# zoltanmaric/h264-fer

Hardware: AMD Instinct MI355X
Metric: macroblocks/sec encode (1080p full-search ME) + bit-exact bitstream vs ref (higher is better)
Workload: dtype u8; 1 GPU; 1080p IPPP encode, full-search +-16 ME (BASELINE configs[2]); content=textured, coded_size=1920x1072, streams_per_gpu=256, contexts_per_gpu=1, gop=30, qp=12, window=32, maxdiff=3, parallelism=1 x 256 independent closed-GOP streams

## Files before the change

### h264-fer_amd/csrc/fer_me.hip

```cpp
#include <stdlib.h>
#include "fer_internal.h"
#include "fer_mvpred.h"

#define INF_M 1000000000

struct WList {
    int m;
    int xy;
};

__device__ __forceinline__ int pack_xy(int x, int y) { return (x & 0xffff) | (y << 16); }
__device__ __forceinline__ int unp_x(int xy) { return (int)(short)(xy & 0xffff); }
__device__ __forceinline__ int unp_y(int xy) { return xy >> 16; }

__device__ __forceinline__ void wl_insert(WList &L, int K, int lane, bool valid, int m, int xy)
{
    int thr = lane_bcast(L.m, K - 1);
    unsigned long long mask = __ballot(valid && m < thr);
    while (mask) {
        int src = __ffsll((long long)mask) - 1;
        mask &= mask - 1;
        int cm = lane_bcast(m, src), cxy = lane_bcast(xy, src);
        int pos = __popcll(__ballot(lane < K && L.m <= cm));
        if (pos < K) {
            int um = FER_DPP(L.m, DPP_WAVE_SHR1), uxy = FER_DPP(L.xy, DPP_WAVE_SHR1);
            if (lane > pos && lane < K) {
                L.m = um;
                L.xy = uxy;
            } else if (lane == pos) {
                L.m = cm;
                L.xy = cxy;
            }
        }
    }
}

#define WAVE_LDS_SYNC()                                    \
    do {                                                   \
        __builtin_amdgcn_fence(__ATOMIC_SEQ_CST, "wavefront"); \
        __builtin_amdgcn_wave_barrier();                   \
    } while (0)
__device__ __forceinline__ int lds_rank64(const unsigned *p, unsigned mine, int n4 = 16)
{
    const uint4 *q = (const uint4 *)p;
    int r = 0;
#pragma unroll 4
    for (int i = 0; i < n4; i++) {
        uint4 k = q[i];
        r += (int)(k.x < mine) + (int)(k.y < mine) + (int)(k.z < mine) + (int)(k.w < mine);
    }
    return r;
}

template <int NB, bool ORDERED, class RAW, class FIN, class ARR>
__device__ __forceinline__ bool select_topk_ex(const int (&v)[NB], int K, int lane, int *sel, WList &L, RAW raw, FIN fin, ARR arr)
{
    unsigned *A = (unsigned *)sel, *B = A + 64;
    int *Ci = sel + 128, *Di = sel + 192;
    const unsigned long long lt = (1ull << lane) - 1ull;
    int lmin = 0x7fffffff, lmax = -1, total = 0;
#pragma unroll
    for (int u = 0; u < NB; u++) {
        total += __popcll(__ballot(v[u] >= 0));
        lmin = (int)min((unsigned)lmin, (unsigned)v[u]);
        lmax = max(lmax, v[u]);
    }
    const int need = min(K, total);
    L.m = INF_M;
    L.xy = 0;
    if (need == 0) return true;
    int c = 65;
    if (!__any(lmax >= (1 << 26))) {
        B[lane] = 0xffffffffu;
        int T0 = 0x7fffffff;
        if (__popcll(__ballot(lmin != 0x7fffffff)) >= need) {
            int lo = 0, hi = (1 << 21) - 1;
            if (__popcll(__ballot(lmin <= hi)) >= need) {
                while (lo < hi) {
                    const int mid = (lo + hi) >> 1;
                    if (__popcll(__ballot(lmin <= mid)) >= need)
                        hi = mid;
                    else
                        lo = mid + 1;
                }
                T0 = lo;
            } else {
                T0 = 1 << 21;
            }
        }
        WAVE_LDS_SYNC();
        if (T0 < (1 << 21) && NB * 64 <= 2048) {
            int nsurv = 0;
#pragma unroll
            for (int u = 0; u < NB; u++) {
                const bool take = (unsigned)v[u] <= (unsigned)T0;
                const unsigned long long mk = __ballot(take);
                if (mk) {
                    const int slot = nsurv + (int)__builtin_amdgcn_mbcnt_hi((uint32_t)(mk >> 32), __builtin_amdgcn_mbcnt_lo((uint32_t)mk, 0u));
                    if (take && slot < 64) {
                        B[slot] = ((unsigned)v[u] << 11) | (unsigned)arr(u);
                        Ci[slot] = raw(u);
                    }
                    nsurv += __popcll(mk);
                }
            }
            WAVE_LDS_SYNC();
            c = nsurv;
        }
    }
    if (c <= 64) {
        WAVE_LDS_SYNC();
        const unsigned mine = B[lane];
        const int mypay = Ci[lane];
        const int rk = lds_rank64(B, mine, (__builtin_amdgcn_readfirstlane(c) + 3) >> 2);
        WAVE_LDS_SYNC();
        if (lane < c && rk < need) {
            A[rk] = mine >> 11;
            Di[rk] = mypay;
        }
        WAVE_LDS_SYNC();
        if (lane < need) {
            L.m = (int)A[lane];
            L.xy = fin(Di[lane]);
        }
        WAVE_LDS_SYNC();
        return true;
    }
    if (!ORDERED) return false;
    int *key = sel, *kxy = sel + 64, *key2 = sel + 128, *kxy2 = sel + 192;
    int lo = wave_min(lmin), hi;
    if (__popcll(__ballot(lmin != 0x7fffffff)) >= need)
        hi = wave_max(lmin != 0x7fffffff ? lmin : -1);
    else
        hi = wave_max(lmax);
    while (lo < hi) {
        int mid = lo + ((hi - lo) >> 1);
        int cnt = 0;
#pragma unroll
        for (int u = 0; u < NB; u++) cnt += __popcll(__ballot(v[u] >= 0 && v[u] <= mid));
        if (cnt >= need)
            hi = mid;
        else
            lo = mid + 1;
    }
    const int T = lo;
    int c_less = 0;
#pragma unroll
    for (int u = 0; u < NB; u++) c_less += __popcll(__ballot(v[u] >= 0 && v[u] < T));
    const int take_eq = need - c_less;
    int nsel = 0, eq_seen = 0;
    WAVE_LDS_SYNC();
#pragma unroll
    for (int u = 0; u < NB; u++) {
        bool ok = v[u] >= 0;
        bool eq = ok && v[u] == T;
        unsigned long long meq = __ballot(eq);
        bool take = (ok && v[u] < T) || (eq && eq_seen + __popcll(meq & lt) < take_eq);
        unsigned long long mt = __ballot(take);
        if (take) {
            int pos = nsel + __popcll(mt & lt);
            key[pos] = v[u];
            kxy[pos] = raw(u);
        }
        nsel += __popcll(mt);
        eq_seen += __popcll(meq);
    }
    WAVE_LDS_SYNC();
    int mk = lane < need ? key[lane] : INF_M, mxy = lane < need ? kxy[lane] : 0;
    int rank = 0;
    for (int i = 0; i < need; i++) {
        int ki = key[i];
        rank += (ki < mk) || (ki == mk && i < lane);
    }
    if (lane < need) {
        key2[rank] = mk;
        kxy2[rank] = mxy;
    }
    WAVE_LDS_SYNC();
    if (lane < need) {
        L.m = key2[lane];
        L.xy = fin(kxy2[lane]);
    }
    WAVE_LDS_SYNC();
    return true;
}
template <int NB, class RAW, class FIN>
__device__ __forceinline__ void select_topk(const int (&v)[NB], int K, int lane, int *sel, WList &L, RAW raw, FIN fin)
{
    select_topk_ex<NB, true>(v, K, lane, sel, L, raw, fin, [&](int u) { return u * 64 + lane; });
}

typedef unsigned short u16x2_t __attribute__((ext_vector_type(2)));
typedef short i16x2_t __attribute__((ext_vector_type(2)));
__device__ __forceinline__ uint32_t pk_sub16(uint32_t a, uint32_t b)
{
    return __builtin_bit_cast(uint32_t, (u16x2_t)(__builtin_bit_cast(u16x2_t, a) - __builtin_bit_cast(u16x2_t, b)));
}
__device__ __forceinline__ uint32_t pk_abs16(uint32_t a)
{
    i16x2_t x = __builtin_bit_cast(i16x2_t, a), z = {0, 0};
    return __builtin_bit_cast(uint32_t, __builtin_elementwise_max(x, (i16x2_t)(z - x)));
}
struct SuPk {
    uint32_t s01, s23, s4;
    uint32_t d01, d23, d4;
    uint32_t s12, s34;
    uint32_t e12, e34;
};
__device__ __forceinline__ SuPk su_pack(const int s[5])
{
    SuPk p;
    p.s01 = (uint32_t)s[0] | ((uint32_t)s[1] << 16);
    p.s23 = (uint32_t)s[2] | ((uint32_t)s[3] << 16);
    p.s4 = (uint32_t)s[4];
    p.d01 = (uint32_t)(s[0] - s[1]) << 16;
    p.d23 = (uint32_t)(s[0] - s[2]) | ((uint32_t)(s[0] - s[3]) << 16);
    p.d4 = (uint32_t)(s[0] - s[4]);
    p.s12 = (uint32_t)s[1] | ((uint32_t)s[2] << 16);
    p.s34 = (uint32_t)s[3] | ((uint32_t)s[4] << 16);
    p.e12 = (uint32_t)(s[0] - s[1]) | ((uint32_t)(s[0] - s[2]) << 16);
    p.e34 = (uint32_t)(s[0] - s[3]) | ((uint32_t)(s[0] - s[4]) << 16);
    return p;
}
__device__ __forceinline__ int feat_dist_w(uint32_t a, uint32_t b, uint32_t c, const SuPk &p)
{
    uint32_t t = __builtin_amdgcn_sad_u16(a, p.s01, 0);
    t = __builtin_amdgcn_sad_u16(b, p.s23, t);
    t = __builtin_amdgcn_sad_u16(c, p.s4, t);
    uint32_t kk = __builtin_amdgcn_perm(a, a, 0x01000100);
    t = __builtin_amdgcn_sad_u16(pk_sub16(kk, a), p.d01, t);
    t = __builtin_amdgcn_sad_u16(pk_sub16(kk, b), p.d23, t);
    t = __builtin_amdgcn_sad_u16(pk_sub16(kk, c) & 0xffffu, p.d4, t);
    return (int)t;
}
__device__ __forceinline__ int feat_dist_rec(const uint16_t *__restrict__ rec, const SuPk &p)
{
    const uint32_t *r = (const uint32_t *)rec;
    return feat_dist_w(r[0], r[1], r[2], p);
}
struct FeatRec {
    uint32_t a, b, c;
};

__device__ __forceinline__ FeatRec feat_rec_direct(const IPlanes &ip, int W, int H, int frac, int refy, int refx)
{
    const int y = iclamp(refy, 0, H - 1), x = iclamp(refx, 0, W - 1);
    const uint8_t *p0 = ip.base + (size_t)frac * ip.plane + (size_t)y * ip.pitch + (x & ~3);
    const uint32_t sh = (uint32_t)(x & 3);
    uint32_t h84[8], hc[8];
#pragma unroll
    for (int r = 0; r < 8; r++) {
        const uint32_t *w = (const uint32_t *)(p0 + (size_t)r * ip.pitch);
        const uint32_t lo = __builtin_amdgcn_alignbyte(w[1], w[0], sh), hi = __builtin_amdgcn_alignbyte(w[2], w[1], sh);
        const uint32_t a4 = __builtin_amdgcn_sad_u8(lo, 0u, 0u);
        h84[r] = __builtin_amdgcn_sad_u8(hi, 0u, a4) | (a4 << 16);
        hc[r] = __builtin_amdgcn_udot4(hi, 0x00000101u, __builtin_amdgcn_udot4(lo, 0x00000101u, 0u, false), false);
    }
    const uint32_t top = h84[0] + h84[1] + h84[2] + h84[3], all = top + h84[4] + h84[5] + h84[6] + h84[7];
    const uint32_t k3 = (h84[0] + h84[1] + h84[4] + h84[5]) & 0xffffu;
    const uint32_t k4 = hc[0] + hc[1] + hc[2] + hc[3] + hc[4] + hc[5] + hc[6] + hc[7];
    FeatRec f;
    f.a = (all & 0xffffu) | (top << 16);
    f.b = (all >> 16) | (k3 << 16);
    f.c = k4;
    return f;
}

template <int R1>
struct LocalGeo {
    static constexpr int N1 = 2 * R1 + 1, PW = 2 * R1 + 8, NC = N1 * N1 * 16, NB = (NC + 63) / 64;
    static constexpr int HTAB = 8 * PW * N1 * 2;
};
template <int R1>
struct LocalLoads {
    static constexpr int ROUNDS = (8 * LocalGeo<R1>::PW + 63) / 64;
    uint4 w[2][ROUNDS];
};
template <int R1>
__device__ __forceinline__ void local_request(const IPlanes &ip, int W, int H, int px0, int py0, int lane, LocalLoads<R1> &ld)
{
    using G = LocalGeo<R1>;
    constexpr int N1 = G::N1, PW = G::PW;
#pragma unroll
    for (int half = 0; half < 2; half++)
#pragma unroll
        for (int k = 0; k < LocalLoads<R1>::ROUNDS; k++) ld.w[half][k] = make_uint4(0, 0, 0, 0);
    if (px0 + N1 - 1 < 0 || px0 >= W || py0 + N1 - 1 < 0 || py0 >= H) return;
    const uint8_t *mbase = ip.base - ((size_t)FER_IP_T * ip.pitch + FER_IP_L);
    const uint32_t obase = __umul24((uint32_t)(py0 + FER_IP_T), (uint32_t)ip.pitch) + (uint32_t)((px0 & ~3) + FER_IP_L);
#pragma unroll
    for (int half = 0; half < 2; half++) {
#pragma unroll
        for (int k = 0; k < LocalLoads<R1>::ROUNDS; k++) {
            const int tt = min(k * 64 + lane, 8 * PW - 1);
            const int fl = tt / PW, r = tt - fl * PW;
            typedef uint32_t u32x4_a4 __attribute__((ext_vector_type(4), aligned(4)));
            const u32x4_a4 v = *(const u32x4_a4 *)(mbase + (obase + __umul24((uint32_t)(half * 8 + fl), (uint32_t)ip.plane) + __umul24((uint32_t)r, (uint32_t)ip.pitch)));
            ld.w[half][k] = make_uint4(v.x, v.y, v.z, v.w);
        }
    }
}
template <int R1>
__device__ __forceinline__ void local_metrics(const IPlanes &ip, int W, int H, int px0, int py0, const SuPk &sp, int lane,
                                              uint32_t *htab, int *mtab, int half_lo = 0, int half_hi = 2, const LocalLoads<R1> *pre = nullptr)
{
    using G = LocalGeo<R1>;
    constexpr int N1 = G::N1, PW = G::PW;
    static_assert(PW + 3 <= 16, "the patch row must fit one 16-byte load");
    if (px0 + N1 - 1 < 0 || px0 >= W || py0 + N1 - 1 < 0 || py0 >= H) {
#pragma unroll
        for (int u = 0; u < G::NB; u++) mtab[u * 64 + lane] = -1;
        WAVE_LDS_SYNC();
        return;
    }
    const uint32_t sh = (uint32_t)(px0 & 3);
    const uint8_t *mbase = ip.base - ((size_t)FER_IP_T * ip.pitch + FER_IP_L);
    const uint32_t obase = __umul24((uint32_t)(py0 + FER_IP_T), (uint32_t)ip.pitch) + (uint32_t)((px0 & ~3) + FER_IP_L);
    for (int half = half_lo; half < half_hi; half++) {
#pragma unroll
        for (int t0 = 0; t0 < 8 * PW; t0 += 64) {
            const int t = t0 + lane;
            const int tt = min(t, 8 * PW - 1);
            const int fl = tt / PW, r = tt - fl * PW;
            typedef uint32_t u32x4_a4 __attribute__((ext_vector_type(4), aligned(4)));
            uint4 w;
            if (pre) {
                w = half == 0 ? pre->w[0][t0 / 64] : pre->w[1][t0 / 64];
            } else {
                const u32x4_a4 v = *(const u32x4_a4 *)(mbase + (obase + __umul24((uint32_t)(half * 8 + fl), (uint32_t)ip.plane) + __umul24((uint32_t)r, (uint32_t)ip.pitch)));
                w = make_uint4(v.x, v.y, v.z, v.w);
            }
            const uint32_t b0 = __builtin_amdgcn_alignbyte(w.y, w.x, sh), b1 = __builtin_amdgcn_alignbyte(w.z, w.y, sh),
                           b2 = __builtin_amdgcn_alignbyte(w.w, w.z, sh);
            if (t < 8 * PW) {
                uint32_t *o = htab + (size_t)tt * N1 * 2;
#pragma unroll
                for (int ix = 0; ix < N1; ix++) {
                    const uint32_t lo = ix < 4 ? __builtin_amdgcn_alignbyte(b1, b0, (uint32_t)(ix & 3)) : b1;
                    const uint32_t hi = ix < 4 ? __builtin_amdgcn_alignbyte(b2, b1, (uint32_t)(ix & 3)) : b2;
                    const uint32_t a4 = __builtin_amdgcn_sad_u8(lo, 0u, 0u);
                    o[ix * 2] = __builtin_amdgcn_sad_u8(hi, 0u, a4) | (a4 << 16);
                    o[ix * 2 + 1] = __builtin_amdgcn_udot4(hi, 0x00000101u, __builtin_amdgcn_udot4(lo, 0x00000101u, 0u, false), false);
                }
            }
        }
        WAVE_LDS_SYNC();
        if (lane < 8 * N1) {
            const int fl = lane / N1, ix = lane - fl * N1;
            uint32_t P84[PW + 1], Pc[PW + 1];
            P84[0] = 0;
            Pc[0] = 0;
#pragma unroll
            for (int r = 0; r < PW; r++) {
                const uint2 h = *(const uint2 *)(htab + ((size_t)(fl * PW + r) * N1 + ix) * 2);
                P84[r + 1] = P84[r] + h.x;
                Pc[r + 1] = Pc[r] + h.y;
            }
            const int refx = px0 + ix, wx = iabs(ix - R1) + 4;
            const bool xok = refx >= 0 && refx < W;
#pragma unroll
            for (int iy = 0; iy < N1; iy++) {
                const uint32_t all = P84[iy + 8] - P84[iy];
                const uint32_t k1 = (P84[iy + 4] - P84[iy]) & 0xffffu;
                const uint32_t k3 = ((P84[iy + 2] - P84[iy]) + (P84[iy + 6] - P84[iy + 4])) & 0xffffu;
                const uint32_t k4 = Pc[iy + 8] - Pc[iy];
                const int D = feat_dist_w((all & 0xffffu) | (k1 << 16), (all >> 16) | (k3 << 16), k4, sp);
                const int refy = py0 + iy;
                const int m = (int)__umul24((uint32_t)(wx + iabs(iy - R1)), (uint32_t)D) | ((xok && refy >= 0 && refy < H) ? 0 : -1);
                mtab[((ix * N1 + iy) << 4) + half * 8 + fl] = m;
            }
        }
        WAVE_LDS_SYNC();
    }
    if (half_lo == 0) {
#pragma unroll
        for (int c = G::NC + lane; c < G::NB * 64; c += 64) mtab[c] = -1;
    }
    WAVE_LDS_SYNC();
}

__device__ __forceinline__ FeatRec feat0_load(const uint16_t *__restrict__ F0, int W, int H, int refy, int refx)
{
    int y = iclamp(refy, 0, H - 1), x = iclamp(refx, 0, W - 1);
    const uint32_t *r = (const uint32_t *)((const char *)F0 + (__umul24((uint32_t)y, (uint32_t)W * 12u) + (uint32_t)x * 12u));
    FeatRec f;
    f.a = r[0];
    f.b = r[1];
    f.c = r[2];
    return f;
}

struct SrcBlk {
    uint32_t lo[8], hi[8];
};
__device__ __forceinline__ SrcBlk src_block_load(const uint8_t *__restrict__ Y, int W, int sx, int sy)
{
    SrcBlk b;
#pragma unroll
    for (int r = 0; r < 8; r++) {
        const uint32_t *q = (const uint32_t *)(Y + (size_t)(sy + r) * W + sx);
        b.lo[r] = __builtin_amdgcn_readfirstlane((int)q[0]);
        b.hi[r] = __builtin_amdgcn_readfirstlane((int)q[1]);
    }
    return b;
}
__device__ __forceinline__ int sad_lane(const IPlanes &ip, int W, int H, int sx, int sy, int mvx, int mvy, const SrcBlk &S)
{
    const int xPi = iclamp(sx + (mvx >> 2), 0, W - 1), yPi = iclamp(sy + (mvy >> 2), 0, H - 1);
    const uint32_t sh = (uint32_t)(xPi & 3);
    const uint32_t o0 = __umul24((uint32_t)((mvx & 3) + (mvy & 3) * 4), (uint32_t)ip.plane) + __umul24((uint32_t)yPi, (uint32_t)ip.pitch) + (uint32_t)(xPi & ~3);
    uint32_t w[8][3];
#pragma unroll
    for (int r = 0; r < 8; r++) {
        const uint32_t *a = (const uint32_t *)(ip.base + (o0 + __umul24((uint32_t)r, (uint32_t)ip.pitch)));
        w[r][0] = a[0];
        w[r][1] = a[1];
        w[r][2] = a[2];
    }
    uint32_t sad = 0;
#pragma unroll
    for (int r = 0; r < 8; r++) {
        const uint32_t r0 = __builtin_amdgcn_alignbyte(w[r][1], w[r][0], sh), r1 = __builtin_amdgcn_alignbyte(w[r][2], w[r][1], sh);
        sad = __builtin_amdgcn_sad_u8(r1, S.hi[r], __builtin_amdgcn_sad_u8(r0, S.lo[r], sad));
    }
    return (int)sad;
}

#define ME_WIDE_LDS 1156
#define ME_SEL_NB 25
#ifndef PRE_WAVES
#define PRE_WAVES 5
#endif
template <int WIN>
__global__ __launch_bounds__(64) __attribute__((amdgpu_waves_per_eu(PRE_WAVES, PRE_WAVES))) void k_me_pre(FerDev d)
{
    const int window = WIN ? WIN : d.window;
    __shared__ __attribute__((aligned(16))) int wide_m[ME_WIDE_LDS];
    __shared__ __attribute__((aligned(16))) int sel_lds[448];
    static_assert(LocalGeo<2>::HTAB <= ME_WIDE_LDS && LocalGeo<2>::NB * 64 <= 448, "LDS regions of k_me_pre");
    const int lane = threadIdx.x;
    const int s = blockIdx.y;
    if (d.hdr[s * 4 + 3] != 0) return;
    const unsigned bx = xcd_swizzle(blockIdx.x, gridDim.x);
    const int mb = (int)(bx >> 2), part = (int)(bx & 3);
    const int W = d.W, H = d.H;
    const size_t ysz = d.ysz;
    const uint8_t *Y = d.curY + (size_t)s * ysz;
    const IPlanes ip = ip_stream(d, s);
    const int sx = ((mb % d.mbw) << 4) + (part & 1) * 8, sy = ((mb / d.mbw) << 4) + (part >> 1) * 8;
    const size_t pidx = ((size_t)s * d.nmb + mb) * 4 + part;

#ifdef FER_PROBE
    const bool probe = FER_DBGF(d, 128) && s == 0 && (bx % 997) == 5;
    long long tmark = probe ? wall_clock64() : 0;
#define PP_MARK(k)                                                          \
    if (probe) {                                                            \
        long long now_ = wall_clock64();                                    \
        if (lane == 0) atomicAdd((unsigned long long *)&d.timing[32 + k], (unsigned long long)(now_ - tmark)); \
        tmark = now_;                                                       \
    }
#else
#define PP_MARK(k)
#endif
    constexpr int RRL = (WIN == 16) ? 1 : 2;
    LocalLoads<RRL> ld;
    const bool fast_path = (WIN == 32 || WIN == 16) && !FER_DBGF(d, 3) && !d.basic;
    if (fast_path) local_request<RRL>(ip, W, H, sx - RRL, sy - RRL, lane, ld);
    int px = lane & 7, py = lane >> 3;
    int v = Y[(size_t)(sy + py) * W + sx + px];
    int su[5];
    su[0] = wave_sum(v);
    su[1] = wave_sum(py > 3 ? 0 : v);
    su[2] = wave_sum(px > 3 ? 0 : v);
    su[3] = wave_sum((py & 3) > 1 ? 0 : v);
    su[4] = wave_sum((px & 3) > 1 ? 0 : v);
    if (lane < 5) d.suma[pidx * 5 + lane] = su[lane];
    if (d.basic) {
        if (lane == 0) {
            d.st3n[pidx] = 0;
            d.v0[pidx] = 0;
        }
        return;
    }
    const SuPk sp = su_pack(su);
    PP_MARK(0)

    WList L;
    L.m = INF_M;
    L.xy = 0;
    const int R = window / 2, n = 2 * R + 1;
    const int r2 = window / 16, n2w = 2 * r2 + 1, nloc = n2w * n2w * 16;
    const uint16_t *F0 = d.feat0 + (size_t)s * 6 * ysz;
    const int wb = (n * n + 63) >> 6;
    if ((WIN == 32 || WIN == 16) && !FER_DBGF(d, 3)) {
        constexpr int WCH = 6;
        constexpr int NN = (WIN ? WIN : 32) + 1;
        constexpr int NBc = WIN ? WIN : 32, RPB = 64 / NBc, NWB = (NN + RPB - 1) / RPB;
        constexpr int LB = LocalGeo<RRL>::NB;
        static_assert(LB <= 7, "ME_SEL_NB leaves room for 7 local batches");
        const int ix = lane % NBc, r0 = lane / NBc;
        const int rx = sx - R + ix;
        const bool xok = rx >= 0 && rx < W;
        const int wx = iabs(ix - R) + 4;
        const uint32_t colo = (uint32_t)iclamp(rx, 0, W - 1) * 12u, rowb = (uint32_t)W * 12u;
        auto fin = [&](int idx) {
            if (idx < wb * 64) return pack_xy((idx / n - R) * 4, (idx % n - R) * 4);
            int c = idx - wb * 64;
            int frac = c & 15, pos = c >> 4;
            return pack_xy((pos / n2w - r2) * 4 + (frac & 3), (pos % n2w - r2) * 4 + (frac >> 2));
        };
        uint32_t k0w[NWB];
#pragma unroll
        for (int b2 = 0; b2 < NWB; b2++) {
            const int ry = iclamp(sy - R + b2 * RPB + r0, 0, H - 1);
            k0w[b2] = *(const uint32_t *)((const char *)F0 + (colo + __umul24((uint32_t)ry, rowb)));
        }
        const uint32_t k0c = feat0_load(F0, W, H, sy - R + min(lane, NN - 1), sx + R).a;
        local_metrics<RRL>(ip, W, H, sx - r2, sy - r2, sp, lane, (uint32_t *)wide_m, sel_lds, 0, 2, &ld);
        int vloc[LB];
        unsigned lminl = 0xffffffffu;
#pragma unroll
        for (int u = 0; u < LB; u++) {
            vloc[u] = sel_lds[u * 64 + lane];
            lminl = min(lminl, (unsigned)vloc[u]);
        }
        int T = 0x7fffffff;
        if (__popcll(__ballot(lminl < (1u << 21))) >= 33) {
            int lo = 0, hi = (1 << 21) - 1;
            while (lo < hi) {
                const int mid = (lo + hi) >> 1;
                if (__popcll(__ballot(lminl <= (unsigned)mid)) >= 33)
                    hi = mid;
                else
                    lo = mid + 1;
            }
            T = lo;
        }
        int *surv = wide_m;
        int ns = 0;
        const uint32_t s0 = (uint32_t)su[0];
        bool done = false;
        if (T != 0x7fffffff) {
#pragma unroll
            for (int b2 = 0; b2 < NWB; b2++) {
                const int iy = b2 * RPB + r0;
                const int ry = sy - R + iy;
                const uint32_t lb = __umul24(5u * (uint32_t)(wx + iabs(iy - R)), __builtin_amdgcn_sad_u16(k0w[b2] & 0xffffu, s0, 0u));
                const bool take = xok && ry >= 0 && ry < H && iy < NN && lb <= (uint32_t)T;
                const unsigned long long mk = __ballot(take);
                if (mk) {
                    const int slot = ns + (int)__builtin_amdgcn_mbcnt_hi((uint32_t)(mk >> 32), __builtin_amdgcn_mbcnt_lo((uint32_t)mk, 0u));
                    if (take && slot < 128) surv[slot] = ix * NN + iy;
                    ns += __popcll(mk);
                }
            }
            {
                const int iy = lane, ry = sy - R + iy;
                const uint32_t lb = __umul24(5u * (uint32_t)(R + 4 + iabs(iy - R)), __builtin_amdgcn_sad_u16(k0c & 0xffffu, s0, 0u));
                const bool take = iy < NN && sx + R < W && ry >= 0 && ry < H && lb <= (uint32_t)T;
                const unsigned long long mk = __ballot(take);
                if (mk) {
                    const int slot = ns + (int)__builtin_amdgcn_mbcnt_hi((uint32_t)(mk >> 32), __builtin_amdgcn_mbcnt_lo((uint32_t)mk, 0u));
                    if (take && slot < 128) surv[slot] = (NN - 1) * NN + iy;
                    ns += __popcll(mk);
                }
            }
            WAVE_LDS_SYNC();
            if (ns <= 128) {
                int v[2 + LB], ar[2];
#pragma unroll
                for (int b2 = 0; b2 < 2; b2++) {
                    v[b2] = -1;
                    ar[b2] = 0;
                    if (b2 * 64 < ns) {
                        const int idx = b2 * 64 + lane;
                        const bool on = idx < ns;
                        const int ai = on ? surv[idx] : 0;
                        const int cix = ai / NN, ciy = ai - cix * NN;
                        const FeatRec f = feat0_load(F0, W, H, sy - R + ciy, sx - R + cix);
                        const int m = (int)__umul24((uint32_t)(iabs(cix - R) + iabs(ciy - R) + 4), (uint32_t)feat_dist_w(f.a, f.b, f.c, sp));
                        v[b2] = on ? m : -1;
                        ar[b2] = ai;
                    }
                }
#pragma unroll
                for (int u = 0; u < LB; u++) v[2 + u] = vloc[u];
                WAVE_LDS_SYNC();
                auto arrv = [&](int u) { return u < 2 ? ar[u < 2 ? u : 0] : wb * 64 + (u - 2) * 64 + lane; };
                done = select_topk_ex<2 + LB, false>(v, 33, lane, sel_lds, L, arrv, fin, arrv);
            }
        }
        PP_MARK(1)
#ifdef FER_STATS
        if (lane == 0) {
            atomicAdd((unsigned long long *)&d.timing[48], 1ull);
            atomicAdd((unsigned long long *)&d.timing[49], done ? 0ull : 1ull);
            atomicAdd((unsigned long long *)&d.timing[50], (unsigned long long)ns);
            atomicAdd((unsigned long long *)&d.timing[51], T == 0x7fffffff ? 1ull : 0ull);
            atomicAdd((unsigned long long *)&d.timing[52], (unsigned long long)(T == 0x7fffffff ? 0 : T));
        }
#endif
        if (!done) {
            WAVE_LDS_SYNC();
            auto wide_load = [&](int iy0, FeatRec (&fr)[WCH]) {
#pragma unroll
                for (int q = 0; q < WCH; q++) {
                    int ry = iclamp(sy - R + iy0 + q * RPB + r0, 0, H - 1);
                    const uint32_t *r = (const uint32_t *)((const char *)F0 + (colo + __umul24((uint32_t)ry, rowb)));
                    fr[q].a = r[0];
                    fr[q].b = r[1];
                    fr[q].c = r[2];
                }
            };
            auto wide_eval = [&](int iy0, const FeatRec (&fr)[WCH]) {
#pragma unroll
                for (int q = 0; q < WCH; q++) {
                    const int iy = iy0 + q * RPB + r0;
                    const int ry = sy - R + iy;
                    const int m = (int)__umul24((uint32_t)(wx + iabs(iy - R)), (uint32_t)feat_dist_w(fr[q].a, fr[q].b, fr[q].c, sp));
                    const int bad = (xok && ry >= 0 && ry < H) ? 0 : -1;
                    wide_m[iy < n ? ix * n + iy : ME_WIDE_LDS - 1] = m | bad;
                }
            };
            {
                constexpr int STEP = RPB * WCH;
                FeatRec fa[WCH], fb[WCH];
                wide_load(0, fa);
                for (int iy0 = 0; iy0 < n; iy0 += 2 * STEP) {
                    if (iy0 + STEP < n) wide_load(iy0 + STEP, fb);
                    wide_eval(iy0, fa);
                    if (iy0 + STEP < n) {
                        if (iy0 + 2 * STEP < n) wide_load(iy0 + 2 * STEP, fa);
                        wide_eval(iy0 + STEP, fb);
                    }
                }
            }
            {
                const int iy = min(lane, n - 1);
                const int rxl = sx + R, ry = sy - R + iy;
                FeatRec f = feat0_load(F0, W, H, ry, rxl);
                int m = (R + 4 + iabs(iy - R)) * feat_dist_w(f.a, f.b, f.c, sp);
                if (!(rxl < W && ry >= 0 && ry < H)) m = -1;
                if (lane < n) wide_m[(n - 1) * n + iy] = m;
            }
            __syncthreads();
            int v[ME_SEL_NB];
#pragma unroll
            for (int u = 0; u < ME_SEL_NB; u++) {
                v[u] = -1;
                if (u < wb) {
                    int c = u * 64 + lane;
                    if (c < n * n) v[u] = wide_m[c];
                } else if (u - wb < LB) {
                    v[u] = vloc[u - wb < LB ? u - wb : 0];
                }
            }
            WAVE_LDS_SYNC();
            auto raw = [&](int u) { return u * 64 + lane; };
            PP_MARK(2)
            select_topk<ME_SEL_NB>(v, 33, lane, sel_lds, L, raw, fin);
        }
        PP_MARK(3)
    } else {
        for (int base = 0; base < n * n && !FER_DBGF(d, 1); base += 64) {
            int c = base + lane;
            int tx = c / n - R, ty = c % n - R;
            int rx = sx + tx, ry = sy + ty;
            bool ok = c < n * n && rx >= 0 && rx < W && ry >= 0 && ry < H;
            int m = 0;
            if (ok) m = (iabs(tx) + iabs(ty) + 4) * feat_dist_rec(F0 + ((size_t)ry * W + rx) * 6, sp);
            wl_insert(L, 33, lane, ok, m, pack_xy(tx * 4, ty * 4));
        }
        for (int base = 0; base < nloc && !FER_DBGF(d, 2); base += 64) {
            int c = base + lane;
            int frac = c & 15, pos = c >> 4;
            int tx = pos / n2w - r2, ty = pos % n2w - r2;
            int rx = sx + tx, ry = sy + ty;
            bool ok = c < nloc && rx >= 0 && rx < W && ry >= 0 && ry < H;
            int m = 0;
            if (ok) {
                const FeatRec f = feat_rec_direct(ip, W, H, frac, ry, rx);
                m = (iabs(tx) + iabs(ty) + 4) * feat_dist_w(f.a, f.b, f.c, sp);
            }
            wl_insert(L, 33, lane, ok, m, pack_xy(tx * 4 + (frac & 3), ty * 4 + (frac >> 2)));
        }
    }
    const int n3 = __popcll(__ballot(lane < 33 && L.m < 100000000));
    int v0 = 0;
    if (!FER_DBGF(d, 4)) {
        const SrcBlk SB = src_block_load(Y, W, sx, sy);
        const int cx = unp_x(L.xy), cy = unp_y(L.xy);
        const int sad = sad_lane(ip, W, H, sx, sy, lane < n3 ? cx : 0, lane < n3 ? cy : 0, SB);
        if (lane < n3) {
            int *o = d.st3 + (pidx * 33 + lane) * 3;
            o[0] = cx;
            o[1] = cy;
            o[2] = sad;
        }
        const int wk = wave_min(lane < n3 ? (sad << 6) | lane : 0x7fffffff);
        if (wk != 0x7fffffff) v0 = lane_bcast(L.xy, wk & 63);
    }
    if (lane == 0) {
        d.st3n[pidx] = n3;
        d.v0[pidx] = v0;
    }

}

__device__ __forceinline__ bool wave_mask_bit(unsigned long long m) { return __builtin_amdgcn_inverse_ballot_w64(m); }
__device__ __forceinline__ unsigned long long wave_ballot(bool p) { return __builtin_amdgcn_ballot_w64(p); }
struct NoProbe {
    __device__ __forceinline__ int operator()(int) const { return 0; }
};
template <bool QUIRK, class SINK, class PROBE = NoProbe>
__device__ __forceinline__ int walk_buckets_q(const FerDev &d, int s, const int (&su)[5], const SuPk &sp, int sx, int sy, int lane,
                                              uint32_t *tbl, int halt_cnt, int &jend, SINK sink, uint32_t max_slice = 0xffffffffu,
                                              bool skip0 = false, PROBE probe = PROBE())
{
    int tren = 0;
    jend = 180;
    const int kt = d.kt;
    const uint32_t *kol2 = d.kol2 + (size_t)s * 16384 * kt;
    const uint32_t *srec = d.sort_rec;
    const int n0 = QUIRK ? d.zero_cnt[s] : 0;
    const uint32_t npos = (uint32_t)(d.W * d.H), g0 = (uint32_t)s * npos;
    const uint16_t *F0 = d.feat0 + (size_t)s * 6 * d.ysz;
    const int t_lo = QUIRK ? 0 : (max(sx - 279, 0) >> d.ktw_shift), t_hi = QUIRK ? kt - 1 : (min(sx + 279, d.W - 1) >> d.ktw_shift);
    auto qstart = [&](int a) -> uint32_t {
        if (a <= 0) return g0;
        if (a == 1) return g0 + min(2u * (uint32_t)n0, npos);
        if (a >= 16384) return g0 + npos;
        return kol2[(size_t)a * kt] - (uint32_t)n0;
    };
    const uint32_t sxy = ((uint32_t)sx << 16) | (uint32_t)sy;
    const char *srec_s = (const char *)(srec + (size_t)g0 * 3);
    auto fetch = [&](unsigned b_start, int b_cnt, uint32_t &r0, uint32_t &r1, uint32_t &r2) {
        const uint32_t li = (b_start - g0) + (unsigned)min(lane, max(b_cnt - 1, 0));
        const uint32_t *e = (const uint32_t *)(srec_s + __umul24(li, 12u));
        r0 = e[0];
        r1 = e[1];
        r2 = e[2];
    };
    auto passes = [&](uint32_t r0, uint32_t r1) -> bool {
        uint32_t dist = __builtin_amdgcn_sad_u16(r0, sxy, 0);
        uint32_t e12 = pk_abs16(pk_sub16(r1, sp.s12));
        return dist < 280u && (pk_sub16(e12, 0x00640064u) & 0x80008000u) == 0x80008000u;
    };
    auto passes_mask = [&](uint32_t r0, uint32_t r1) -> unsigned long long {
        uint32_t dist = __builtin_amdgcn_sad_u16(r0, sxy, 0);
        uint32_t e12 = pk_abs16(pk_sub16(r1, sp.s12));
        return wave_ballot(dist < 280u) & wave_ballot((pk_sub16(e12, 0x00640064u) & 0x80008000u) == 0x80008000u);
    };
    auto feat_d = [&](uint32_t info, uint32_t r0, uint32_t r1, uint32_t r2) -> uint32_t {
        uint32_t D;
        if (!QUIRK) {
            const uint32_t aa = ((info >> 16) & 0x7fffu) * 0x10001u;
            D = __builtin_amdgcn_sad_u16(r1, sp.s12, (info >> 8) & 255u);
            D = __builtin_amdgcn_sad_u16(r2, sp.s34, D);
            D = __builtin_amdgcn_sad_u16(pk_sub16(aa, r1), sp.e12, D);
            D = __builtin_amdgcn_sad_u16(pk_sub16(aa, r2), sp.e34, D);
        } else {
            int px = min((int)(r0 >> 16), d.W - 1), py = min((int)(r0 & 0xffff), d.H - 1);
            D = (uint32_t)feat_dist_rec(F0 + ((size_t)py * d.W + px) * 6, sp);
        }
        return D;
    };
    auto filter = [&](uint32_t info, uint32_t r0, uint32_t r1, uint32_t r2) -> bool {
        const int b_cnt = (int)(info & 127u);
        bool ok = lane < b_cnt && passes(r0, r1);
        unsigned long long mk = __ballot(ok);
        int rank = tren + (int)__builtin_amdgcn_mbcnt_hi((uint32_t)(mk >> 32), __builtin_amdgcn_mbcnt_lo((uint32_t)mk, 0u));
        const uint32_t D = feat_d(info, r0, r1, r2);
        const bool halt = sink(ok, rank, (int)pk_sub16(r0, sxy), (int)D, info, false);
        tren += __popcll(mk);
        return halt || tren > halt_cnt;
    };
    auto run_table = [&](uint32_t dstart, uint32_t dinfo, int nb) -> bool {
        auto desc = [&](int b, unsigned &bs, uint32_t &bi) {
            const int bb = min(b, 63);
            bs = (unsigned)__builtin_amdgcn_readlane((int)dstart, bb);
            bi = (uint32_t)__builtin_amdgcn_readlane((int)dinfo, bb);
        };
        unsigned sA, sB, sC, sD;
        uint32_t iA, iB, iC, iD;
        uint32_t A0, A1, A2, B0, B1, B2, C0, C1, C2, D0, D1, D2;
        desc(0, sA, iA);
        fetch(sA, (int)(iA & 127u), A0, A1, A2);
        desc(1, sB, iB);
        fetch(sB, (int)(iB & 127u), B0, B1, B2);
        desc(2, sC, iC);
        fetch(sC, (int)(iC & 127u), C0, C1, C2);
        desc(3, sD, iD);
        fetch(sD, (int)(iD & 127u), D0, D1, D2);
#define WALK_STEP(SS, II, R0, R1, R2, NEXT)                                  \
        if (filter(II, R0, R1, R2)) {       \
            jend = (int)((II >> 8) & 255u);                                  \
            return true;                                                     \
        }                                                                    \
        if (II & 128u) {                                                     \
            if (tren > 128) {                                                \
                jend = (int)((II >> 8) & 255u);                              \
                return true;                                                 \
            }                                                                \
        }                                                                    \
        desc(NEXT, SS, II);                                                  \
        fetch(SS, (int)(II & 127u), R0, R1, R2);
        for (int b = 0; b < nb; b += 4) {
            WALK_STEP(sA, iA, A0, A1, A2, b + 4)
            if (b + 1 >= nb) break;
            WALK_STEP(sB, iB, B0, B1, B2, b + 5)
            if (b + 2 >= nb) break;
            WALK_STEP(sC, iC, C0, C1, C2, b + 6)
            if (b + 3 >= nb) break;
            WALK_STEP(sD, iD, D0, D1, D2, b + 7)
        }
#undef WALK_STEP
        return false;
    };
    for (int j0 = 0; j0 <= 180; j0 += 16) {
        uint32_t kb = 0u;
        {
            const int which = lane >> 4, jj = j0 + (lane & 15);
            const int a = (which & 2) ? su[0] + jj : su[0] - jj;
            const bool va = a >= 0 && a < 16384 && jj <= 180;
            if (!QUIRK) {
                if (va) kb = kol2[(size_t)a * kt + ((which & 1) ? t_hi + 1 : t_lo)];
            } else {
                if (va) kb = qstart(a + (which & 1));
            }
        }
        const int step = (lane >> 1) & 15, side = lane & 1;
        const uint32_t st = (uint32_t)__shfl((int)kb, step + (side ? 32 : 0)), en = (uint32_t)__shfl((int)kb, step + (side ? 48 : 16));
        uint32_t cnt = (lane < 32 && en > st) ? en - st : 0u;
        if (cnt > max_slice && (j0 + step > 0 || skip0)) cnt = 0u;
        const int a_k = side ? su[0] + j0 + step : su[0] - (j0 + step);
        const uint32_t ja = ((uint32_t)(j0 + step) << 8) | ((uint32_t)(a_k & 0x7fff) << 16) | ((uint32_t)side << 31);
        int pre = (int)cnt;
#pragma unroll
        for (int o = 1; o < 32; o <<= 1) {
            int v = __shfl_up(pre, o);
            if (lane >= o) pre += v;
        }
        const int T = __builtin_amdgcn_readlane(pre, 31);
        if (T == 0) continue;
        if (T <= 62 * 64) {
            const uint32_t E = (uint32_t)pre - cnt;
            const uint32_t cnt_hi = (uint32_t)__shfl((int)cnt, lane | 1);
            const bool closes = side == 1 || cnt_hi == 0u;
            const unsigned long long ne = __ballot(cnt > 0u);
            const int nne = __popcll(ne);
            const int rk = (int)__builtin_amdgcn_mbcnt_hi((uint32_t)(ne >> 32), __builtin_amdgcn_mbcnt_lo((uint32_t)ne, 0u));
            WAVE_LDS_SYNC();
            tbl[lane] = 0u;
            tbl[64 + lane] = 0u;
            WAVE_LDS_SYNC();
            if (cnt > 0u) {
                __hip_atomic_fetch_or(&tbl[E >> 5], 1u << (E & 31u), __ATOMIC_RELAXED, __HIP_MEMORY_SCOPE_WAVEFRONT);
                tbl[128 + 2 * rk] = st - E - g0;
                tbl[129 + 2 * rk] = ja | (closes ? 128u : 0u);
            }
            if (lane == 0) __hip_atomic_fetch_or(&tbl[T >> 5], 1u << (T & 31), __ATOMIC_RELAXED, __HIP_MEMORY_SCOPE_WAVEFRONT);
            WAVE_LDS_SYNC();
            const int nbd = (T + 63) >> 6;
            int dbase = 0;
            auto ddesc = [&](int b, uint32_t &li, uint32_t &inf) {
                const int bb = min(b, nbd - 1);
                const uint32_t w0 = tbl[2 * bb], w1 = tbl[2 * bb + 1];
                const unsigned long long M = ((unsigned long long)w1 << 32) | w0;
                const int inc = (int)__builtin_amdgcn_mbcnt_hi(w1, __builtin_amdgcn_mbcnt_lo(w0, 0u)) + (int)((M >> lane) & 1ull);
                const int r = min(dbase + inc - 1, nne - 1);
                dbase += __popcll(M);
                const uint32_t g = min(64u * (uint32_t)bb + (uint32_t)lane, (uint32_t)T - 1u);
                const uint2 e = *(const uint2 *)&tbl[128 + 2 * r];
                li = b < nbd ? e.x + g : 0u;
                inf = e.y;
            };
            auto fetchl = [&](uint32_t li, uint32_t &r0, uint32_t &r1, uint32_t &r2) {
                const uint32_t *e = (const uint32_t *)(srec_s + __umul24(li, 12u));
                r0 = e[0];
                r1 = e[1];
                r2 = e[2];
            };
            const int stop_lim = min(128, halt_cnt);
            auto dstep = [&](int b, uint32_t inf, uint32_t r0, uint32_t r1, uint32_t r2) -> bool {
                const int rem = T - 64 * b;
                unsigned long long vm = ~0ull, mk = passes_mask(r0, r1);
                if (rem < 64) {
                    vm = (1ull << rem) - 1ull;
                    mk &= vm;
                }
                const int nmk = __popcll(mk);
                const int rank = tren + (int)__builtin_amdgcn_mbcnt_hi((uint32_t)(mk >> 32), __builtin_amdgcn_mbcnt_lo((uint32_t)mk, 0u));
                const int rel = (int)pk_sub16(r0, sxy), D = (int)feat_d(inf, r0, r1, r2);
                if (tren + nmk <= stop_lim) {
                    const bool halt = sink(wave_mask_bit(mk), rank, rel, D, inf, true);
                    tren += nmk;
                    const unsigned long long hm = wave_ballot(halt);
                    if (hm) {
                        jend = __builtin_amdgcn_readlane((int)((inf >> 8) & 255u), __ffsll((long long)hm) - 1);
                        return true;
                    }
                    return false;
                }
                const int incl = rank + (int)wave_mask_bit(mk);
                const int jl = (int)((inf >> 8) & 255u);
                const unsigned long long M = ((unsigned long long)__builtin_amdgcn_readfirstlane((int)tbl[2 * b + 1]) << 32) |
                                             (uint32_t)__builtin_amdgcn_readfirstlane((int)tbl[2 * b]);
                const unsigned long long lastm = (M >> 1) | ((unsigned long long)(__builtin_amdgcn_readfirstlane((int)tbl[2 * b + 2]) & 1) << 63);
                const unsigned long long s1 = wave_ballot((inf & 128u) != 0u) & wave_ballot(incl > 128) & lastm & vm;
                const unsigned long long s2 = wave_ballot(incl > halt_cnt) & vm;
                unsigned long long live = vm;
                if (s1) live &= (2ull << (__ffsll((long long)s1) - 1)) - 1ull;
                if (s2) {
                    const int j2 = __builtin_amdgcn_readlane(jl, __ffsll((long long)s2) - 1);
                    live &= wave_ballot(jl <= j2);
                }
                const bool halt = sink(wave_mask_bit(mk & live), rank, rel, D, inf, false);
                tren += __popcll(mk & live);
                const unsigned long long hm = wave_ballot(halt);
                if (hm) {
                    jend = __builtin_amdgcn_readlane(jl, __ffsll((long long)hm) - 1);
                    return true;
                }
                if (s1 | s2) {
                    jend = __builtin_amdgcn_readlane(jl, 63 - __clzll((long long)live));
                    return true;
                }
                return false;
            };
            uint32_t lA, lB, lC, lD, iA, iB, iC, iD;
            uint32_t A0, A1, A2, B0, B1, B2, C0, C1, C2, D0, D1, D2;
            ddesc(0, lA, iA);
            fetchl(lA, A0, A1, A2);
            ddesc(1, lB, iB);
            fetchl(lB, B0, B1, B2);
            ddesc(2, lC, iC);
            fetchl(lC, C0, C1, C2);
            ddesc(3, lD, iD);
            fetchl(lD, D0, D1, D2);
#define DENSE_STEP(LL, II, R0, R1, R2, B) \
            if (dstep(B, II, R0, R1, R2)) return tren; \
            ddesc(B + 4, LL, II);                     \
            fetchl(LL, R0, R1, R2);
            for (int b = 0; b < nbd; b += 4) {
                DENSE_STEP(lA, iA, A0, A1, A2, b)
                if (b + 1 >= nbd) break;
                DENSE_STEP(lB, iB, B0, B1, B2, b + 1)
                if (b + 2 >= nbd) break;
                DENSE_STEP(lC, iC, C0, C1, C2, b + 2)
                if (b + 3 >= nbd) break;
                DENSE_STEP(lD, iD, D0, D1, D2, b + 3)
            }
#undef DENSE_STEP
        } else {
            for (int k = 0; k < 32; k++) {
                const uint32_t ks = (uint32_t)__builtin_amdgcn_readlane((int)st, k), kc = (uint32_t)__builtin_amdgcn_readlane((int)cnt, k);
                const uint32_t kja = (uint32_t)__builtin_amdgcn_readlane((int)ja, k);
                const int knb = (int)((kc + 63u) >> 6);
                if (kc > (uint32_t)FER_BIG_SLICE) {
                    const int known = probe((int)((kja >> 16) & 0x7fffu));
                    if (known > 0 && tren + known > halt_cnt) {
                        tren += known;
                        jend = j0 + (k >> 1);
                        return tren;
                    }
                }
                for (int b0 = 0; b0 < knb; b0 += 62) {
                    const int m = min(62, knb - b0);
                    const uint32_t off = 64u * (uint32_t)(b0 + lane);
                    const bool on = lane < m;
                    if (run_table(on ? ks + off : g0, on ? (min(kc - off, 64u) | kja) : 0u, m)) return tren;
                }
                if ((k & 1) && tren > 128) {
                    jend = j0 + (k >> 1);
                    return tren;
                }
            }
        }
    }
    return tren;
}

template <class SINK, class PROBE = NoProbe>
__device__ __forceinline__ int walk_buckets(const FerDev &d, int s, const int (&su)[5], const SuPk &sp, int sx, int sy, int lane,
                                            uint32_t *tbl, int halt_cnt, int &jend, SINK sink, PROBE probe = PROBE())
{
    jend = 0;
    if (d.basic || FER_DBGF(d, 8)) return 0;
    if (d.zero_cnt[s] > 0) return walk_buckets_q<true>(d, s, su, sp, sx, sy, lane, tbl, 0x7fffffff, jend, sink);
    return walk_buckets_q<false>(d, s, su, sp, sx, sy, lane, tbl, halt_cnt, jend, sink, 0xffffffffu, false, probe);
}

__global__ __launch_bounds__(64, 8) void k_me_walk(FerDev d)
{
    const int lane = threadIdx.x;
    const int s = blockIdx.y;
    if (d.hdr[s * 4 + 3] != 0) return;
    const int mb = blockIdx.x >> 2, part = blockIdx.x & 3;
    const int W = d.W;
    const uint8_t *Y = d.curY + (size_t)s * d.ysz;
    const int sx = ((mb % d.mbw) << 4) + (part & 1) * 8, sy = ((mb / d.mbw) << 4) + (part >> 1) * 8;
    const size_t pidx = ((size_t)s * d.nmb + mb) * 4 + part;
    int px = lane & 7, py = lane >> 3;
    int v = Y[(size_t)(sy + py) * W + sx + px];
    int su[5];
    su[0] = wave_sum(v);
    su[1] = wave_sum(py > 3 ? 0 : v);
    su[2] = wave_sum(px > 3 ? 0 : v);
    su[3] = wave_sum((py & 3) > 1 ? 0 : v);
    su[4] = wave_sum((px & 3) > 1 ? 0 : v);
    const SuPk sp = su_pack(su);
    int2 *out = (int2 *)(d.st2 + pidx * FER_ST2_CAP * 2);
    __shared__ __attribute__((aligned(16))) uint32_t tbl[192];
// ... 953 lines not shown
```

Baseline: 22.04 million macroblocks/s.

## Cut register pressure in k_me_pre to raise occupancy to seven waves

Raises the k_me_pre occupancy target from 5 to 7 waves per EU and reduces live state to fit. The second half of the local patch loads is now issued lazily through a hook inside local_metrics, so it is not held in registers for the whole call. A LEAN mode computes the k4 window sums on the fly rather than keeping a full prefix array. WCH drops from 6 to 3, vloc is reloaded from LDS only when it is needed, LDS is merged into one region, and the survivor ballot uses precomputed row and column masks. The tighter register budget may cause spills or less latency hiding inside each wave, and reusing LDS regions risks aliasing mistakes.

```diff
diff --git a/h264-fer_amd/csrc/fer_me.hip b/h264-fer_amd/csrc/fer_me.hip
--- a/h264-fer_amd/csrc/fer_me.hip
+++ b/h264-fer_amd/csrc/fer_me.hip
@@ -277,19 +277,22 @@
     uint4 w[2][ROUNDS];
 };
 template <int R1>
-__device__ __forceinline__ void local_request(const IPlanes &ip, int W, int H, int px0, int py0, int lane, LocalLoads<R1> &ld)
+__device__ __forceinline__ void local_request(const IPlanes &ip, int W, int H, int px0, int py0, int lane, LocalLoads<R1> &ld,
+                                              int half_lo = 0, int half_hi = 2)
 {
     using G = LocalGeo<R1>;
     constexpr int N1 = G::N1, PW = G::PW;
 #pragma unroll
     for (int half = 0; half < 2; half++)
 #pragma unroll
-        for (int k = 0; k < LocalLoads<R1>::ROUNDS; k++) ld.w[half][k] = make_uint4(0, 0, 0, 0);
+        for (int k = 0; k < LocalLoads<R1>::ROUNDS; k++)
+            if (half >= half_lo && half < half_hi) ld.w[half][k] = make_uint4(0, 0, 0, 0);
     if (px0 + N1 - 1 < 0 || px0 >= W || py0 + N1 - 1 < 0 || py0 >= H) return;
     const uint8_t *mbase = ip.base - ((size_t)FER_IP_T * ip.pitch + FER_IP_L);
     const uint32_t obase = __umul24((uint32_t)(py0 + FER_IP_T), (uint32_t)ip.pitch) + (uint32_t)((px0 & ~3) + FER_IP_L);
 #pragma unroll
     for (int half = 0; half < 2; half++) {
+        if (half < half_lo || half >= half_hi) continue;
 #pragma unroll
         for (int k = 0; k < LocalLoads<R1>::ROUNDS; k++) {
             const int tt = min(k * 64 + lane, 8 * PW - 1);
@@ -300,9 +303,13 @@
         }
     }
 }
-template <int R1>
+struct NoHook {
+    __device__ __forceinline__ void operator()(int) const {}
+};
+template <int R1, class HOOK = NoHook, bool LEAN = false>
 __device__ __forceinline__ void local_metrics(const IPlanes &ip, int W, int H, int px0, int py0, const SuPk &sp, int lane,
-                                              uint32_t *htab, int *mtab, int half_lo = 0, int half_hi = 2, const LocalLoads<R1> *pre = nullptr)
+                                              uint32_t *htab, int *mtab, int half_lo = 0, int half_hi = 2, const LocalLoads<R1> *pre = nullptr,
+                                              HOOK hook = HOOK())
 {
     using G = LocalGeo<R1>;
     constexpr int N1 = G::N1, PW = G::PW;
@@ -317,6 +324,7 @@
     const uint8_t *mbase = ip.base - ((size_t)FER_IP_T * ip.pitch + FER_IP_L);
     const uint32_t obase = __umul24((uint32_t)(py0 + FER_IP_T), (uint32_t)ip.pitch) + (uint32_t)((px0 & ~3) + FER_IP_L);
     for (int half = half_lo; half < half_hi; half++) {
+        hook(half);
 #pragma unroll
         for (int t0 = 0; t0 < 8 * PW; t0 += 64) {
             const int t = t0 + lane;
@@ -347,14 +355,20 @@
         WAVE_LDS_SYNC();
         if (lane < 8 * N1) {
             const int fl = lane / N1, ix = lane - fl * N1;
-            uint32_t P84[PW + 1], Pc[PW + 1];
+            uint32_t P84[PW + 1], Pc[LEAN ? 1 : PW + 1], k4l[N1];
             P84[0] = 0;
             Pc[0] = 0;
 #pragma unroll
             for (int r = 0; r < PW; r++) {
                 const uint2 h = *(const uint2 *)(htab + ((size_t)(fl * PW + r) * N1 + ix) * 2);
                 P84[r + 1] = P84[r] + h.x;
-                Pc[r + 1] = Pc[r] + h.y;
+                if constexpr (LEAN) {
+                    if (r < N1) k4l[r] = Pc[0];
+                    Pc[0] += h.y;
+                    if (r >= 7) k4l[r - 7] = Pc[0] - k4l[r - 7];
+                } else {
+                    Pc[r + 1] = Pc[r] + h.y;
+                }
             }
             const int refx = px0 + ix, wx = iabs(ix - R1) + 4;
             const bool xok = refx >= 0 && refx < W;
@@ -363,7 +377,11 @@
                 const uint32_t all = P84[iy + 8] - P84[iy];
                 const uint32_t k1 = (P84[iy + 4] - P84[iy]) & 0xffffu;
                 const uint32_t k3 = ((P84[iy + 2] - P84[iy]) + (P84[iy + 6] - P84[iy + 4])) & 0xffffu;
-                const uint32_t k4 = Pc[iy + 8] - Pc[iy];
+                uint32_t k4;
+                if constexpr (LEAN)
+                    k4 = k4l[iy];
+                else
+                    k4 = Pc[iy + 8] - Pc[iy];
                 const int D = feat_dist_w((all & 0xffffu) | (k1 << 16), (all >> 16) | (k3 << 16), k4, sp);
                 const int refy = py0 + iy;
                 const int m = (int)__umul24((uint32_t)(wx + iabs(iy - R1)), (uint32_t)D) | ((xok && refy >= 0 && refy < H) ? 0 : -1);
@@ -426,18 +444,25 @@
     return (int)sad;
 }
 
+__device__ __forceinline__ bool wave_mask_bit(unsigned long long m) { return __builtin_amdgcn_inverse_ballot_w64(m); }
+__device__ __forceinline__ unsigned long long wave_ballot(bool p) { return __builtin_amdgcn_ballot_w64(p); }
+
 #define ME_WIDE_LDS 1156
+#define ME_ROW_LDS 960
+#define ME_PRE_LDS 1408
 #define ME_SEL_NB 25
 #ifndef PRE_WAVES
-#define PRE_WAVES 5
+#define PRE_WAVES 7
 #endif
 template <int WIN>
 __global__ __launch_bounds__(64) __attribute__((amdgpu_waves_per_eu(PRE_WAVES, PRE_WAVES))) void k_me_pre(FerDev d)
 {
     const int window = WIN ? WIN : d.window;
-    __shared__ __attribute__((aligned(16))) int wide_m[ME_WIDE_LDS];
-    __shared__ __attribute__((aligned(16))) int sel_lds[448];
-    static_assert(LocalGeo<2>::HTAB <= ME_WIDE_LDS && LocalGeo<2>::NB * 64 <= 448, "LDS regions of k_me_pre");
+    __shared__ __attribute__((aligned(16))) int pre_lds[ME_PRE_LDS];
+    int *const wide_m = pre_lds, *const sel_lds = pre_lds + ME_ROW_LDS;
+    static_assert(LocalGeo<2>::HTAB <= ME_ROW_LDS && LocalGeo<2>::NB * 64 <= ME_PRE_LDS - ME_ROW_LDS && ME_WIDE_LDS <= ME_PRE_LDS &&
+                      128 + 256 <= ME_ROW_LDS && 256 <= ME_PRE_LDS - ME_ROW_LDS && ME_ROW_LDS % 4 == 0,
+                  "LDS regions of k_me_pre");
     const int lane = threadIdx.x;
     const int s = blockIdx.y;
     if (d.hdr[s * 4 + 3] != 0) return;
@@ -465,7 +490,7 @@
     constexpr int RRL = (WIN == 16) ? 1 : 2;
     LocalLoads<RRL> ld;
     const bool fast_path = (WIN == 32 || WIN == 16) && !FER_DBGF(d, 3) && !d.basic;
-    if (fast_path) local_request<RRL>(ip, W, H, sx - RRL, sy - RRL, lane, ld);
+    if (fast_path) local_request<RRL>(ip, W, H, sx - RRL, sy - RRL, lane, ld, 0, 1);
     int px = lane & 7, py = lane >> 3;
     int v = Y[(size_t)(sy + py) * W + sx + px];
     int su[5];
@@ -493,7 +518,7 @@
     const uint16_t *F0 = d.feat0 + (size_t)s * 6 * ysz;
     const int wb = (n * n + 63) >> 6;
     if ((WIN == 32 || WIN == 16) && !FER_DBGF(d, 3)) {
-        constexpr int WCH = 6;
+        constexpr int WCH = 3;
         constexpr int NN = (WIN ? WIN : 32) + 1;
         constexpr int NBc = WIN ? WIN : 32, RPB = 64 / NBc, NWB = (NN + RPB - 1) / RPB;
         constexpr int LB = LocalGeo<RRL>::NB;
@@ -516,14 +541,13 @@
             k0w[b2] = *(const uint32_t *)((const char *)F0 + (colo + __umul24((uint32_t)ry, rowb)));
         }
         const uint32_t k0c = feat0_load(F0, W, H, sy - R + min(lane, NN - 1), sx + R).a;
-        local_metrics<RRL>(ip, W, H, sx - r2, sy - r2, sp, lane, (uint32_t *)wide_m, sel_lds, 0, 2, &ld);
-        int vloc[LB];
+        auto second_group = [&](int half) {
+            if (half == 0) local_request<RRL>(ip, W, H, sx - RRL, sy - RRL, lane, ld, 1, 2);
+        };
+        local_metrics<RRL, decltype(second_group), true>(ip, W, H, sx - r2, sy - r2, sp, lane, (uint32_t *)wide_m, sel_lds, 0, 2, &ld, second_group);
         unsigned lminl = 0xffffffffu;
 #pragma unroll
-        for (int u = 0; u < LB; u++) {
-            vloc[u] = sel_lds[u * 64 + lane];
-            lminl = min(lminl, (unsigned)vloc[u]);
-        }
+        for (int u = 0; u < LB; u++) lminl = min(lminl, (unsigned)sel_lds[u * 64 + lane]);
         int T = 0x7fffffff;
         if (__popcll(__ballot(lminl < (1u << 21))) >= 33) {
             int lo = 0, hi = (1 << 21) - 1;
@@ -541,27 +565,35 @@
         const uint32_t s0 = (uint32_t)su[0];
         bool done = false;
         if (T != 0x7fffffff) {
+            static_assert((NBc / 2) % RPB == 0 && NN <= 64, "a batch stays on one side of the centre row");
+            const int iy_lo = max(0, R - sy), iy_hi = min(NN - 1, H - 1 - (sy - R));
+            const unsigned long long rowv = ((2ull << iy_hi) - 1ull) & ~((1ull << iy_lo) - 1ull);
+            const unsigned long long colv = wave_ballot(xok);
+            constexpr unsigned long long GRP = NBc == 64 ? ~0ull : (1ull << NBc) - 1ull;
+            const uint32_t w5lo = 5u * (uint32_t)(wx + R - r0), w5hi = 5u * (uint32_t)(wx - R + r0);
+            const int arr0 = ix * NN + r0;
 #pragma unroll
             for (int b2 = 0; b2 < NWB; b2++) {
-                const int iy = b2 * RPB + r0;
-                const int ry = sy - R + iy;
-                const uint32_t lb = __umul24(5u * (uint32_t)(wx + iabs(iy - R)), __builtin_amdgcn_sad_u16(k0w[b2] & 0xffffu, s0, 0u));
-                const bool take = xok && ry >= 0 && ry < H && iy < NN && lb <= (uint32_t)T;
-                const unsigned long long mk = __ballot(take);
+                unsigned long long valid = 0;
+#pragma unroll
+                for (int j = 0; j < RPB; j++)
+                    if ((rowv >> (b2 * RPB + j)) & 1ull) valid |= GRP << (j * NBc);
+                valid &= colv;
+                const uint32_t w5 = b2 * RPB < R ? w5lo - 5u * (uint32_t)(b2 * RPB) : w5hi + 5u * (uint32_t)(b2 * RPB);
+                const uint32_t lb = __umul24(w5, __builtin_amdgcn_sad_u16(k0w[b2] & 0xffffu, s0, 0u));
+                const unsigned long long mk = wave_ballot(lb <= (uint32_t)T) & valid;
                 if (mk) {
                     const int slot = ns + (int)__builtin_amdgcn_mbcnt_hi((uint32_t)(mk >> 32), __builtin_amdgcn_mbcnt_lo((uint32_t)mk, 0u));
-                    if (take && slot < 128) surv[slot] = ix * NN + iy;
+                    if (wave_mask_bit(mk) && slot < 128) surv[slot] = arr0 + b2 * RPB;
                     ns += __popcll(mk);
                 }
             }
             {
-                const int iy = lane, ry = sy - R + iy;
-                const uint32_t lb = __umul24(5u * (uint32_t)(R + 4 + iabs(iy - R)), __builtin_amdgcn_sad_u16(k0c & 0xffffu, s0, 0u));
-                const bool take = iy < NN && sx + R < W && ry >= 0 && ry < H && lb <= (uint32_t)T;
-                const unsigned long long mk = __ballot(take);
+                const uint32_t lb = __umul24(5u * (uint32_t)(R + 4 + iabs(lane - R)), __builtin_amdgcn_sad_u16(k0c & 0xffffu, s0, 0u));
+                const unsigned long long mk = sx + R < W ? wave_ballot(lb <= (uint32_t)T) & rowv : 0ull;
                 if (mk) {
                     const int slot = ns + (int)__builtin_amdgcn_mbcnt_hi((uint32_t)(mk >> 32), __builtin_amdgcn_mbcnt_lo((uint32_t)mk, 0u));
-                    if (take && slot < 128) surv[slot] = (NN - 1) * NN + iy;
+                    if (wave_mask_bit(mk) && slot < 128) surv[slot] = (NN - 1) * NN + lane;
                     ns += __popcll(mk);
                 }
             }
@@ -584,10 +616,10 @@
                     }
                 }
 #pragma unroll
-                for (int u = 0; u < LB; u++) v[2 + u] = vloc[u];
+                for (int u = 0; u < LB; u++) v[2 + u] = sel_lds[u * 64 + lane];
                 WAVE_LDS_SYNC();
                 auto arrv = [&](int u) { return u < 2 ? ar[u < 2 ? u : 0] : wb * 64 + (u - 2) * 64 + lane; };
-                done = select_topk_ex<2 + LB, false>(v, 33, lane, sel_lds, L, arrv, fin, arrv);
+                done = select_topk_ex<2 + LB, false>(v, 33, lane, wide_m + 128, L, arrv, fin, arrv);
             }
         }
         PP_MARK(1)
@@ -601,6 +633,10 @@
         }
 #endif
         if (!done) {
+            WAVE_LDS_SYNC();
+            int vloc[LB];
+#pragma unroll
+            for (int u = 0; u < LB; u++) vloc[u] = sel_lds[u * 64 + lane];
             WAVE_LDS_SYNC();
             auto wide_load = [&](int iy0, FeatRec (&fr)[WCH]) {
 #pragma unroll
@@ -707,8 +743,6 @@
 
 }
 
-__device__ __forceinline__ bool wave_mask_bit(unsigned long long m) { return __builtin_amdgcn_inverse_ballot_w64(m); }
-__device__ __forceinline__ unsigned long long wave_ballot(bool p) { return __builtin_amdgcn_ballot_w64(p); }
 struct NoProbe {
     __device__ __forceinline__ int operator()(int) const { return 0; }
 };
```

Result: faster. 22.78 million macroblocks/s (median of 6 runs) (+3.4%).
